# Berghojo/bmhrl

Measured on AMD Instinct MI355X. Metric: caption-train steps/sec, higher is better.
Workload: dtype bf16; 1 GPU; BMHRL warmstart step (BASELINE configs[1]): B=16/GPU Tv=256 Ta=800 L=30 V=10172 N=2 d_model=1024 H=4 dropout=0.1; global_batch=16, parallelism=dp1, launch=hip-graph

## Files before the change

bmhrl_amd/csrc/gemm.hip:

```cpp
#include <cstdlib>
#include <algorithm>
#include <type_traits>

#include "common.h"
#include "../../include/bmhrl_hip.h"

namespace {

struct GemmArgs {
  int M, N, K, batch2;
  const bf16_t* A; long lda, a_sb1, a_sb2;
  const bf16_t* B; long ldb, b_sb1, b_sb2;
  float* C; long ldc, c_sb1, c_sb2;
  bf16_t* Cb; long ldcb, cb_sb1, cb_sb2;
  int epilogue; float alpha; int relu; int accumulate;
  const float* bias;
  const float* residual; long ldr, r_sb1, r_sb2;
  const uint8_t* mask; long mask_sb1, mask_sm;
  const float* rowvec; const float* rowvec2; long rv_sb1, rv_sb2;
  const bf16_t* aux; long ldaux, aux_sb1, aux_sb2;
  float dropout_p; uint64_t seed; const uint64_t* seed_dev; long drop_sb1, drop_sb2, drop_sm;
  float* colsum; long cs_sb2, bias_sb2, cs_sb1, bias_sb1;
  int tiles_m, splits, k_per_split, vec_ok, dbg, fast_bf16, fast_pd, fast_f32, tiles_mn;
  int xcd_chunk, group_m;
// ... 586 lines not shown
}

struct GemmGroup {
  GemmArgs p0, p1, p2, p3;
  int first[5];
  int n;
};
template <int TM, int TN, bool AT, bool BT>
__global__ __launch_bounds__(256, 2) void gemm_group_kernel(const GemmGroup g) {
  const int b = (int)blockIdx.x;
  int i = 0;
  if (g.n > 1 && b >= g.first[1]) i = 1;
  if (g.n > 2 && b >= g.first[2]) i = 2;
  if (g.n > 3 && b >= g.first[3]) i = 3;
  GemmArgs p = g.p0;
  if (i == 1) p = g.p1;
  if (i == 2) p = g.p2;
  if (i == 3) p = g.p3;
  int r = b - g.first[i];
  const int bx = r % p.tiles_mn;
  r /= p.tiles_mn;
  gemm_body<TM, TN, AT, BT>(p, bx, r % p.splits, r / p.splits);
}


template <int N> struct IC { static constexpr int value = N; };
template <int I, int N, class F>
__device__ __forceinline__ void gsfor(F&& f) {
  if constexpr (I < N) {
    f(IC<I>{});
    gsfor<I + 1, N>(f);
  }
}
template <int IMM>
__device__ __forceinline__ void gemm_glds16(const char* src, char* dst) {
  __builtin_amdgcn_global_load_lds((const __attribute__((address_space(1))) void*)src,
                                   (__attribute__((address_space(3))) void*)dst, 16, IMM, 0);
}

template <int OFF>
__device__ __forceinline__ bf16x8 gemm_lds128(unsigned addr) {
  bf16x8 r;
  asm volatile("ds_read_b128 %0, %1 offset:%2" : "=v"(r) : "v"(addr), "n"(OFF));
  return r;
}
template <int OFF>
__device__ __forceinline__ bf16x4 gemm_ldstr(unsigned addr) {
  bf16x4 r;
  asm volatile("ds_read_b64_tr_b16 %0, %1 offset:%2" : "=v"(r) : "v"(addr), "n"(OFF));
  return r;
}

template <int TM, int TN, bool AT, bool BT, int NS>
__global__ __launch_bounds__(256, 2) void gemm_glds_kernel(const GemmArgs p) {
  constexpr int BM = 64 * TM, BN = 64 * TN;
  constexpr int A_BYTES = BM * BK * 2, B_BYTES = BN * BK * 2, STAGE_BYTES = A_BYTES + B_BYTES;
  constexpr int EPI_ELEMS = BM * (BN + 4) * 2;
  constexpr int SMEM_ELEMS = (NS * STAGE_BYTES / 2) > EPI_ELEMS ? (NS * STAGE_BYTES / 2) : EPI_ELEMS;

  __shared__ __attribute__((aligned(16))) bf16_t smem[SMEM_ELEMS];
  char* const sbase = reinterpret_cast<char*>(smem);
  const unsigned lds0 = (unsigned)(uintptr_t)(__attribute__((address_space(3))) char*)sbase;

  const int tid = threadIdx.x, lane = tid & 63;
  const int wave = __builtin_amdgcn_readfirstlane(tid >> 6);
  const int wm = wave >> 1, wn = wave & 1;
  const int r32 = lane & 31, h = lane >> 5;
  const int g1 = (lane >> 4) & 1, q4 = (lane & 15) >> 2, p4 = lane & 3;
  const int bz = blockIdx.z, b1 = bz / p.batch2, b2 = bz % p.batch2;
  int tile_m, tile_n;
  tile_of_block(p, (int)blockIdx.x, tile_m, tile_n);
  const int m0 = tile_m * BM, n0 = tile_n * BN;
  const char* __restrict__ Ag = reinterpret_cast<const char*>(p.A + b1 * p.a_sb1 + b2 * p.a_sb2);
  const char* __restrict__ Bg = reinterpret_cast<const char*>(p.B + b1 * p.b_sb1 + b2 * p.b_sb2);
  const int M8 = (p.M + 7) & ~7, N8 = (p.N + 7) & ~7;
  const int k_begin = blockIdx.y * p.k_per_split;
  const int k_end = min(p.K, k_begin + p.k_per_split);
  const int nk = (k_end - k_begin) / BK;
  if (nk <= 0) return;
  BMHRL_GSTAMP(0)

  constexpr int PA = A_BYTES / 1024 / 4, PB = B_BYTES / 1024 / 4;
  unsigned a_off[PA], b_off[PB];
  auto piece_off = [&](const bool trans, const int R, const int i, const int r0, const int rmax, const int rmax8, const long ld) {
    if (!trans) {
      const int row = wave * (R / 4) + 8 * i + (lane >> 3), pc = lane & 7;
      const int sc = pc ^ ((row >> 1) & 7);
      return (unsigned)((long)min(r0 + row, rmax - 1) * ld * 2 + sc * 16);
    }
    const int cpr = R / 8, rpp = 64 / cpr;
    const int krow = wave * 16 + rpp * i + lane / cpr, pc = lane % cpr;
    const int sc = pc ^ (R == 128 ? ((krow & 3) << 2) : (((krow >> 1) & 1) << 2));
    return (unsigned)((long)krow * ld * 2 + (long)min(r0 + sc * 8, rmax8 - 8) * 2);
  };
#pragma unroll
  for (int i = 0; i < PA; ++i) a_off[i] = piece_off(AT, BM, i, m0, p.M, M8, p.lda);
#pragma unroll
  for (int i = 0; i < PB; ++i) b_off[i] = piece_off(BT, BN, i, n0, p.N, N8, p.ldb);
  const long a_step = AT ? (long)BK * p.lda * 2 : (long)BK * 2, b_step = BT ? (long)BK * p.ldb * 2 : (long)BK * 2;
  const char* const a_k0 = Ag + (AT ? (long)k_begin * p.lda * 2 : (long)k_begin * 2);
  const char* const b_k0 = Bg + (BT ? (long)k_begin * p.ldb * 2 : (long)k_begin * 2);
  char* const a_dst = sbase + wave * PA * 1024;
  char* const b_dst = sbase + A_BYTES + wave * PB * 1024;
  auto stage = [&](auto st_, const int t) {
    constexpr int ST = decltype(st_)::value;
    auto sgpr_ptr = [](const char* q) {
      const uint64_t u = reinterpret_cast<uint64_t>(q);
      const uint32_t lo = __builtin_amdgcn_readfirstlane((uint32_t)u), hi = __builtin_amdgcn_readfirstlane((uint32_t)(u >> 32));
      return reinterpret_cast<const char*>(((uint64_t)hi << 32) | lo);
    };
    const char* ab = sgpr_ptr(a_k0 + (long)t * a_step);
    const char* bb = sgpr_ptr(b_k0 + (long)t * b_step);
    gsfor<0, PA>([&](auto i) {
      constexpr int I = decltype(i)::value;
      unsigned o = a_off[I];
      asm volatile("" : "+v"(o));
      gemm_glds16<0>(ab + o, a_dst + ST * STAGE_BYTES + I * 1024);
    });
    gsfor<0, PB>([&](auto i) {
      constexpr int I = decltype(i)::value;
      unsigned o = b_off[I];
      asm volatile("" : "+v"(o));
      gemm_glds16<0>(bb + o, b_dst + ST * STAGE_BYTES + I * 1024);
    });
  };

  constexpr int NA = AT ? TM : 4, NB = BT ? TN : 4;
  unsigned a_addr0[NA], b_addr0[NB];
  if constexpr (!AT) {
// ... 64 lines not shown
    read_ks(IC<1>{});
    gsfor<0, 4>([&](auto ks_) {
      constexpr int KS = decltype(ks_)::value;
      constexpr int LEFT = KS < 3 ? PER_KS : 0;
      __builtin_amdgcn_sched_barrier(0);
      bf16x8& a0 = af[KS][0];
      bf16x8& b0 = bfr[KS][0];
      bf16x8& a1 = af[KS][TM - 1];
      bf16x8& b1r = bfr[KS][TN - 1];
      if constexpr (TM == 2 && TN == 2) asm volatile("s_waitcnt lgkmcnt(%4)" : "+v"(a0), "+v"(a1), "+v"(b0), "+v"(b1r) : "n"(LEFT));
      else asm volatile("s_waitcnt lgkmcnt(%2)" : "+v"(a0), "+v"(b0) : "n"(LEFT));
      __builtin_amdgcn_sched_barrier(0);
#pragma unroll
      for (int mi = 0; mi < TM; ++mi)
#pragma unroll
        for (int ni = 0; ni < TN; ++ni)
          acc[mi][ni] = __builtin_amdgcn_mfma_f32_32x32x16_bf16(af[KS][mi], bfr[KS][ni], acc[mi][ni], 0, 0, 0);
      if constexpr (KS + 2 < 4) read_ks(IC<KS + 2>{});
    });
  };

  constexpr int PT = PA + PB;
  auto step = [&](auto st_, const int t) {
    constexpr int ST = decltype(st_)::value;
    constexpr int NXT = (ST + NS - 1) % NS;
    const bool more = t + NS - 1 < nk;
    if (more) stage(IC<NXT>{}, t + NS - 1);
    compute(st_);
    if (t + 1 < nk) {
      if (more && NS > 2) asm volatile("s_waitcnt vmcnt(%0)" ::"n"((NS - 2) * PT) : "memory");
      else asm volatile("s_waitcnt vmcnt(0)" ::: "memory");
      __builtin_amdgcn_s_barrier();
      asm volatile("" ::: "memory");
    }
  };
  gsfor<0, NS - 1>([&](auto i_) {
    if (decltype(i_)::value < nk) stage(i_, decltype(i_)::value);
  });
  BMHRL_GSTAMP(1)
  if (NS > 2 && nk > 1) asm volatile("s_waitcnt vmcnt(%0)" ::"n"((NS - 2) * PT) : "memory");
  if (NS == 2 || nk < NS - 1) asm volatile("s_waitcnt vmcnt(0)" ::: "memory");
  __builtin_amdgcn_s_barrier();
  asm volatile("" ::: "memory");
  BMHRL_GSTAMP(2)
  for (int t0 = 0; t0 < nk; t0 += NS) {
    gsfor<0, NS>([&](auto i_) {
      if (t0 + decltype(i_)::value < nk) step(i_, t0 + decltype(i_)::value);
    });
  }
  asm volatile("s_waitcnt lgkmcnt(0)" ::: "memory");
  __builtin_amdgcn_s_barrier();
  asm volatile("" ::: "memory");
  BMHRL_GSTAMP(3)
  gemm_epilogue<TM, TN, SMEM_ELEMS>(p, acc, smem, b1, b2, m0, n0, (int)blockIdx.y);
  BMHRL_GSTAMP(4)
}

template <bool AT, bool BT>
__global__ __launch_bounds__(512, 2) void gemm_glds8_kernel(const GemmArgs p) {
  constexpr int TM = 2, TN = 2, NS = 3, NW = 8;
  constexpr int BM = 128, BN = 128;
  constexpr int A_BYTES = BM * BK * 2, B_BYTES = BN * BK * 2, STAGE_BYTES = A_BYTES + B_BYTES;
  constexpr int EPI_ELEMS = BM * (BN + 4) * 2;
  constexpr int SMEM_ELEMS = (NS * STAGE_BYTES / 2) > EPI_ELEMS ? (NS * STAGE_BYTES / 2) : EPI_ELEMS;
  static_assert(4 * 64 * 256 <= SMEM_ELEMS * 2, "the partial tile of wave group 1 fits the stages");

  __shared__ __attribute__((aligned(16))) bf16_t smem[SMEM_ELEMS];
  char* const sbase = reinterpret_cast<char*>(smem);
  const unsigned lds0 = (unsigned)(uintptr_t)(__attribute__((address_space(3))) char*)sbase;

  const int tid = threadIdx.x, lane = tid & 63;
  const int wave = __builtin_amdgcn_readfirstlane(tid >> 6);
  const int grp = wave >> 2, w4 = wave & 3;
  const int wm = w4 >> 1, wn = w4 & 1;
  const int r32 = lane & 31, h = lane >> 5;
  const int g1 = (lane >> 4) & 1, q4 = (lane & 15) >> 2, p4 = lane & 3;
  const int bz = blockIdx.z, b1 = bz / p.batch2, b2 = bz % p.batch2;
  const int tile_m = blockIdx.x % p.tiles_m, tile_n = blockIdx.x / p.tiles_m;
  const int m0 = tile_m * BM, n0 = tile_n * BN;
  const char* __restrict__ Ag = reinterpret_cast<const char*>(p.A + b1 * p.a_sb1 + b2 * p.a_sb2);
  const char* __restrict__ Bg = reinterpret_cast<const char*>(p.B + b1 * p.b_sb1 + b2 * p.b_sb2);
  const int M8 = (p.M + 7) & ~7, N8 = (p.N + 7) & ~7;
  const int nk = p.K / BK;
  BMHRL_GSTAMP(0)

  constexpr int PA = A_BYTES / 1024 / NW, PB = B_BYTES / 1024 / NW;
  unsigned a_off[PA], b_off[PB];
  auto piece_off = [&](const bool trans, const int R, const int i, const int r0, const int rmax, const int rmax8, const long ld) {
    if (!trans) {
      const int row = wave * (R / NW) + 8 * i + (lane >> 3), pc = lane & 7;
      const int sc = pc ^ ((row >> 1) & 7);
      return (unsigned)((long)min(r0 + row, rmax - 1) * ld * 2 + sc * 16);
    }
    const int cpr = R / 8, rpp = 64 / cpr;
    const int krow = wave * (64 / NW) + rpp * i + lane / cpr, pc = lane % cpr;
    const int sc = pc ^ ((krow & 3) << 2);
    return (unsigned)((long)krow * ld * 2 + (long)min(r0 + sc * 8, rmax8 - 8) * 2);
  };
#pragma unroll
  for (int i = 0; i < PA; ++i) a_off[i] = piece_off(AT, BM, i, m0, p.M, M8, p.lda);
#pragma unroll
  for (int i = 0; i < PB; ++i) b_off[i] = piece_off(BT, BN, i, n0, p.N, N8, p.ldb);
  const long a_step = AT ? (long)BK * p.lda * 2 : (long)BK * 2, b_step = BT ? (long)BK * p.ldb * 2 : (long)BK * 2;
  char* const a_dst = sbase + wave * PA * 1024;
  char* const b_dst = sbase + A_BYTES + wave * PB * 1024;
  auto stage = [&](auto st_, const int t) {
    constexpr int ST = decltype(st_)::value;
    auto sgpr_ptr = [](const char* q) {
// ... 357 lines not shown
             d->r_sb2 % 4 == 0 && al(d->aux, 8) && d->ldaux % 4 == 0 && d->aux_sb1 % 4 == 0 && d->aux_sb2 % 4 == 0 &&
             al(d->bias, 16) && d->bias_sb2 % 4 == 0 && d->bias_sb1 % 4 == 0;
  a.fast_bf16 = d->Cb && !d->C && d->epilogue == BMHRL_EPI_LINEAR && !d->mask && !d->residual && !d->aux && !d->colsum &&
                !d->accumulate && al(d->Cb, 16) && d->ldcb % 8 == 0 && d->cb_sb1 % 8 == 0 && d->cb_sb2 % 8 == 0;
  static const int fast_f32_on = getenv("BMHRL_GEMM_FAST_F32") ? atoi(getenv("BMHRL_GEMM_FAST_F32")) : 1;
  const bool f32_combo = d->accumulate ? (!d->residual && d->dropout_p == 0.f && !d->Cb)
                                       : d->residual ? (d->dropout_p > 0.f || !d->Cb) : (d->dropout_p == 0.f && !d->Cb);
  a.fast_f32 = fast_f32_on && d->C && d->epilogue == BMHRL_EPI_LINEAR && !d->mask && !d->aux && !d->rowvec && !d->rowvec2 &&
               !d->relu && !d->colsum && f32_combo && a.vec_ok;
  const bool out_ok = d->Cb && !d->C && !d->residual && !d->colsum && !d->accumulate && !d->bias && al(d->Cb, 16) &&
                      d->ldcb % 8 == 0 && d->cb_sb1 % 8 == 0 && d->cb_sb2 % 8 == 0 && d->rowvec;
  a.fast_pd = (d->epilogue == BMHRL_EPI_PROB && out_ok && d->rowvec2 && (!d->mask || d->mask_sm == 0) && !d->aux) ||
              (d->epilogue == BMHRL_EPI_DSCORE && out_ok && d->aux && al(d->aux, 16) && d->ldaux % 8 == 0 &&
               d->aux_sb1 % 8 == 0 && d->aux_sb2 % 8 == 0 && (!d->mask || d->mask_sm == 0));
  const bool can_split = d->allow_split_k && d->C && !d->Cb && d->epilogue == BMHRL_EPI_LINEAR && !d->relu && !d->mask &&
                         d->dropout_p == 0.f && (!d->accumulate || d->split_ws) && !d->colsum;
  tp = tile_plan(d->M, d->N, d->K, batch, can_split);
  a.split_ws = (tp.splits > 1 && d->split_ws && d->split_ws_elems >= (int64_t)tp.splits * batch * d->M * d->N) ? d->split_ws : nullptr;
  if (tp.splits > 1 && d->accumulate && !a.split_ws) return -22;
  return 0;
}

int plan_problem(const bmhrl_gemm_desc* d, GemmArgs& a, GemmPlan& pl, int& batch) {
  TilePlan tp;
  if (const int rc = prepare(d, a, tp, batch)) return rc;
  const int TM = tp.mid || tp.big ? 2 : 1, TN = tp.big && !tp.mid ? 2 : 1;
  pl.tile = tp.mid ? TILE_128x64 : tp.big ? TILE_128 : TILE_64;
  pl.splits = tp.splits;
  pl.loop = LOOP_REG;
  pl.stages = 2;
  if (uses_glds(a, d->a_trans, d->b_trans)) {
    static const int force_ns = getenv("BMHRL_GEMM_STAGES") ? atoi(getenv("BMHRL_GEMM_STAGES")) : 0;
    const long blocks = (long)((d->M + 64 * TM - 1) / (64 * TM)) * ((d->N + 64 * TN - 1) / (64 * TN)) * batch;
    int ns = TM == 1 && tp.splits == 1 && blocks <= 448 ? 4 : 2;
    if (force_ns) ns = TM == 1 ? (force_ns >= 4 ? 4 : 2) : 2;
    pl.loop = LOOP_GLDS;
    pl.stages = ns;
    static const int w8 = getenv("BMHRL_GEMM_W8") ? atoi(getenv("BMHRL_GEMM_W8")) : 0;
    static const long w8_max = getenv("BMHRL_GEMM_W8MAX") ? atol(getenv("BMHRL_GEMM_W8MAX")) : 256;
    if (TM == 2 && TN == 2 && w8 && tp.splits == 1 && d->K >= 2 * BK && (w8 == 2 || blocks <= w8_max)) {
      pl.loop = LOOP_GLDS8;
      pl.stages = 3;
    }
  }
  pl.split_form = tp.splits == 1 ? SPLIT_NONE : a.split_ws ? SPLIT_ORDERED : SPLIT_ATOMIC;
  pl.epi_path = tp.splits == 1 && a.fast_bf16 ? EPIPATH_FAST_BF16 : tp.splits == 1 && a.fast_pd ? EPIPATH_FAST_PD : EPIPATH_GENERIC;
  if (tp.splits != 1 || pl.loop == LOOP_GLDS8) a.fast_f32 = 0;
  pl.fast_f32 = a.fast_f32;
  pl.vec_ok = a.vec_ok;
  pl.ordered_colsum = bmhrl_deterministic() && a.colsum != nullptr;
  return 0;
}

int group_prepare(const bmhrl_gemm_desc* d, int n, GemmGroup& g, int& total) {
  GemmArgs* ps[4] = {&g.p0, &g.p1, &g.p2, &g.p3};
  bool same = n > 1;
  total = 0;
  for (int i = 0; i < n; ++i) {
    GemmPlan pl;
    int batch;
    if (const int rc = plan_problem(d + i, *ps[i], pl, batch)) return rc;
    GemmArgs& p = *ps[i];
    same = same && pl.tile == TILE_64 && pl.loop == LOOP_REG && d[i].a_trans == d[0].a_trans && d[i].b_trans == d[0].b_trans &&
           pl.split_form != SPLIT_ORDERED && !pl.ordered_colsum;
    p.tiles_m = (p.M + 63) / 64;
    p.tiles_mn = p.tiles_m * ((p.N + 63) / 64);
    p.splits = pl.splits;
    p.dbg = 0;
    const int ktiles = (p.K + BK - 1) / BK;
    p.k_per_split = ((ktiles + pl.splits - 1) / pl.splits) * BK;
    g.first[i] = total;
    total += p.tiles_mn * pl.splits * batch;
  }
  return same ? 1 : 0;
}
}

extern "C" int bmhrl_gemm_plan(const bmhrl_gemm_desc* d, int32_t plan[8]) {
  GemmArgs a;
  GemmPlan pl;
  int batch;
  if (const int rc = plan_problem(d, a, pl, batch)) return rc;
  if (plan) {
    plan[0] = pl.loop; plan[1] = pl.tile; plan[2] = pl.stages; plan[3] = pl.splits;
    plan[4] = pl.split_form; plan[5] = pl.epi_path; plan[6] = pl.vec_ok; plan[7] = pl.ordered_colsum;
  }
  return 0;
}

extern "C" int bmhrl_gemm_f32_fast_path(const bmhrl_gemm_desc* d) {
  GemmArgs a;
  GemmPlan pl;
  int batch;
  if (const int rc = plan_problem(d, a, pl, batch)) return rc;
  return pl.fast_f32;
}

extern "C" int bmhrl_gemm_group_plan(const bmhrl_gemm_desc* d, int32_t n) {
  BMHRL_CHECK_ARG(d && n >= 1);
  int launches = 0;
  for (int i = 0; i < n; i += 4) {
    GemmGroup g;
    int total;
    const int rc = group_prepare(d + i, n - i < 4 ? n - i : 4, g, total);
    if (rc < 0) return rc;
    launches += rc;
  }
  return launches;
}

void gemm_trace_dump(const GemmArgs& a, hipStream_t stream) {
#ifdef BMHRL_GEMM_TRACE
  if (getenv("BMHRL_GEMM_TRACE")) {
    long long hh[2][8];
    (void)hipStreamSynchronize(stream);
    (void)hipMemcpyFromSymbol(hh, HIP_SYMBOL(g_gemm_trace), sizeof(hh));
    for (int w = 0; w < 2; ++w)
      fprintf(stderr, "gemm trace (%s block, M %d N %d K %d): setup %lld  first tile %lld  loop %lld  epilogue %lld  total %lld\n",
              w ? "last" : "first", a.M, a.N, a.K, hh[w][1] - hh[w][0], hh[w][2] - hh[w][1], hh[w][3] - hh[w][2], hh[w][4] - hh[w][3],
              hh[w][4] - hh[w][0]);
  }
#else
  (void)a; (void)stream;
#endif
}

extern "C" int bmhrl_gemm(const bmhrl_gemm_desc* d, bmhrl_stream_t stream) {
  GemmArgs a;
  GemmPlan pl;
  int batch;
  if (const int rc = plan_problem(d, a, pl, batch)) return rc;
  GemmArgs full = a;
  if (pl.ordered_colsum) a.colsum = nullptr;
  hipError_t e;
  if (pl.tile == TILE_128x64) e = launch<2, 1>(a, pl, d->a_trans, d->b_trans, batch, (hipStream_t)stream);
  else if (pl.tile == TILE_128) e = launch<2, 2>(a, pl, d->a_trans, d->b_trans, batch, (hipStream_t)stream);
  else e = launch<1, 1>(a, pl, d->a_trans, d->b_trans, batch, (hipStream_t)stream);
  if (e == hipSuccess && pl.ordered_colsum) {
    hipLaunchKernelGGL(colsum_ordered_kernel, dim3((unsigned)((full.N + 63) / 64)), dim3(1024), 0, (hipStream_t)stream, full, d->batch1);
    e = hipGetLastError();
  }
  if (e == hipSuccess && pl.split_form == SPLIT_ORDERED) {
    GemmArgs r = a;
    r.splits = pl.splits;
    const int ktiles = (a.K + BK - 1) / BK, tiles_per_split = (ktiles + pl.splits - 1) / pl.splits;
    const int n_live = (ktiles + tiles_per_split - 1) / tiles_per_split;
    const long total = (long)batch * a.M * a.N;
    hipLaunchKernelGGL(splitk_reduce_kernel, dim3((unsigned)std::min<long>((total + 255) / 256, 2048)), dim3(256), 0, (hipStream_t)stream, r, batch,
                       n_live);
    e = hipGetLastError();
  }
  gemm_trace_dump(a, (hipStream_t)stream);
  return hip_status(e);
}

extern "C" int bmhrl_gemm_group(const bmhrl_gemm_desc* d, int32_t n, bmhrl_stream_t stream) {
  BMHRL_CHECK_ARG(d && n >= 1);
  if (n > 4) {
    for (int i = 0; i < n; i += 4)
      if (const int rc = bmhrl_gemm_group(d + i, n - i < 4 ? n - i : 4, stream)) return rc;
    return 0;
  }
  GemmGroup g;
  int total;
  const int same = group_prepare(d, n, g, total);
  if (same < 0) return same;
  if (!same) {
    for (int i = 0; i < n; ++i)
      if (const int rc = bmhrl_gemm(d + i, stream)) return rc;
    return 0;
  }
  GemmArgs* ps[4] = {&g.p0, &g.p1, &g.p2, &g.p3};
  for (int i = n; i < 5; ++i) g.first[i] = total;
  for (int i = n; i < 4; ++i) *ps[i] = g.p0;
  g.n = n;
  dim3 grid((unsigned)total), block(256);
  const hipStream_t s = (hipStream_t)stream;
  if (!d[0].a_trans && !d[0].b_trans) hipLaunchKernelGGL((gemm_group_kernel<1, 1, false, false>), grid, block, 0, s, g);
  else if (!d[0].a_trans && d[0].b_trans) hipLaunchKernelGGL((gemm_group_kernel<1, 1, false, true>), grid, block, 0, s, g);
  else if (d[0].a_trans && !d[0].b_trans) hipLaunchKernelGGL((gemm_group_kernel<1, 1, true, false>), grid, block, 0, s, g);
  else hipLaunchKernelGGL((gemm_group_kernel<1, 1, true, true>), grid, block, 0, s, g);
  return hip_status(hipGetLastError());
}
```

bmhrl_amd/functional.py:

```python
from __future__ import annotations

import math
import itertools
import os
import weakref
from typing import Optional

import torch

from . import ops
from .ops import pad8

_BF16 = torch.bfloat16


class ShadowCache:

    def __init__(self):
        self.w = {}
        self.b = {}
        self.split = {}
        self.epoch = 0

    def invalidate(self):
# ... 426 lines not shown
    scale = 1.0 / math.sqrt(dk)
    Skp = pad8(Sk)
    pstr = (H * Sq * Skp, Sq * Skp)
    fused = (FUSED_SCORES_BWD and stats[0] == "flash" and ops.attention_bwd_scores256_ok(Sq, Sk, dk, msq)
             and all(v % 8 == 0 for v in (ldq, ldk, ldv, q_off, k_off, v_off)))
    if fused:
        P = torch.empty(B, H, Sq, Skp, dtype=_BF16, device=dev)
        dS = torch.empty(B, H, Sq, Skp, dtype=_BF16, device=dev)
        ops.attention_bwd_scores256(Qb, ldq, Kb, ldk, Vb, ldv, dOb, D, stats[1], stats[2], mask, msb, P, dS, Skp, B, H, Sq, Sk,
                                    scale, q_off=q_off, k_off=k_off, v_off=v_off)
        _attn_grad_products(P, dS, pstr, dOb, Qb, q_off, ldq, Kb, k_off, ldk, dQb, dq_off, lddq, dKb, dk_off, lddk, dVb, dv_off,
                            lddv, B, H, Sq, Sk, dk, Skp, csq, csk, csv)
        return
    delta = torch.empty(B, H, Sq, device=dev)
    ops.attn_delta(dOb, D, Ob, D, delta, B, H, Sq, dk, scale=1.0 - p_drop)
    if stats[0] == "flash":
        P = _padded_bf16(B * H * Sq, Sk, dev).view(B, H, Sq, Skp)
        ops.gemm(Qb, Kb, Sq, Sk, dk, lda=ldq, ldb=ldk, a_off=q_off, b_off=k_off, batch=(B, H), a_strides=(Sq * ldq, dk),
                 b_strides=(Sk * ldk, dk), C_bf16=P, ldcb=Skp, cb_strides=pstr, epilogue=ops.EPI_PROB, alpha=scale,
                 mask=mask, mask_sb1=msb, mask_sm=msq, rowvec=stats[1], rowvec2=stats[2], rv_strides=(H * Sq, Sq))
    else:
        P = stats[1]
    dS = _padded_bf16(B * H * Sq, Sk, dev).view(B, H, Sq, Skp)
    ops.gemm(dOb, Vb, Sq, Sk, dk, lda=D, ldb=ldv, b_off=v_off, batch=(B, H), a_strides=(Sq * D, dk),
             b_strides=(Sk * ldv, dk), C_bf16=dS, ldcb=Skp, cb_strides=pstr, epilogue=ops.EPI_DSCORE, alpha=scale,
             rowvec=delta, rv_strides=(H * Sq, Sq), aux=P, ldaux=Skp, aux_strides=pstr, mask=mask, mask_sb1=msb, mask_sm=msq)
    _attn_grad_products(P, dS, pstr, dOb, Qb, q_off, ldq, Kb, k_off, ldk, dQb, dq_off, lddq, dKb, dk_off, lddk, dVb, dv_off, lddv,
                        B, H, Sq, Sk, dk, Skp, csq, csk, csv)


def _attn_grad_products(P, dS, pstr, dOb, Qb, q_off, ldq, Kb, k_off, ldk, dQb, dq_off, lddq, dKb, dk_off, lddk, dVb, dv_off, lddv,
                        B, H, Sq, Sk, dk, Skp, csq, csk, csv):
    D = H * dk
    ops.gemm(P, dOb, Sk, dk, Sq, lda=Skp, ldb=D, a_trans=True, b_trans=True, batch=(B, H), a_strides=pstr,
             b_strides=(Sq * D, dk), C_bf16=dVb, ldcb=lddv, cb_off=dv_off, cb_strides=(Sk * lddv, dk), **csv)
    ops.gemm(dS, Qb, Sk, dk, Sq, lda=Skp, ldb=ldq, b_off=q_off, a_trans=True, b_trans=True, batch=(B, H), a_strides=pstr,
             b_strides=(Sq * ldq, dk), C_bf16=dKb, ldcb=lddk, cb_off=dk_off, cb_strides=(Sk * lddk, dk), **csk)
    ops.gemm(dS, Kb, Sq, dk, Sk, lda=Skp, ldb=ldk, b_off=k_off, b_trans=True, batch=(B, H), a_strides=pstr,
             b_strides=(Sk * ldk, dk), C_bf16=dQb, ldcb=lddq, cb_off=dq_off, cb_strides=(Sq * lddq, dk), **csq)


ORDERED_DX = os.environ.get("BMHRL_ORDERED_DX", "1") == "1"


def _split_ws(M, N, K, batch, device):
    if not ORDERED_DX:
        return None
    n = ops.gemm_splits(M, N, K, batch)
    return SCRATCH.f32(n * batch * M * N, device=device, zero=False) if n > 1 else None


def _linear_bwd(dyb, ldy, rows, N, xb, ldx, K, wb, *, need_dw, need_db, need_dx, dx_f32=None, dx_bf16=None, lddxb=0,
                dx_epilogue=ops.EPI_LINEAR, dx_alpha=1.0, dx_aux=None, ldaux=0, dx_drop=0.0, dx_seed=0,
                dy_off=0, x_off=0, w_off=0, dx_accumulate=False, dx_colsum=None, dx_split_k=False, leaf=None):
    dev = dyb.device
    dw = db = None
    if need_dw:
        dw = SCRATCH.f32(N, K, device=dev, zero=not ops.gemm_overwrites(N, K, rows))
        ops.gemm(dyb, xb, N, K, rows, lda=ldy, ldb=ldx, a_off=dy_off, b_off=x_off, a_trans=True, b_trans=True, C_f32=dw, ldc=K,
                 allow_split_k=True, defer=leaf)
    if need_db:
        db = SCRATCH.f32(N, device=dev)
        ops.colsum_bf16(dyb, ldy, db, True, rows, N, dy_off=dy_off)
    if need_dx:
        ws = _split_ws(rows, K, N, 1, dev) if dx_split_k else None
        ops.gemm(dyb, wb, rows, K, N, lda=ldy, ldb=wb.shape[1], a_off=dy_off, b_off=w_off, b_trans=True, C_f32=dx_f32,
                 ldc=K, C_bf16=dx_bf16, ldcb=lddxb, epilogue=dx_epilogue, alpha=dx_alpha, aux=dx_aux, ldaux=ldaux,
                 dropout_p=dx_drop, seed=dx_seed, seed_dev=SEEDS.dev, accumulate=dx_accumulate, colsum=dx_colsum,
                 allow_split_k=dx_split_k, split_ws=ws)
    return dw, db


def _row_stride(t, cols):
    if t.dim() < 2 or t.shape[-1] != cols or t.stride(-1) != 1:
        return None
    for i in range(t.dim() - 2):
        if t.shape[i] != 1 and t.stride(i) != t.stride(i + 1) * t.shape[i + 1]:
            return None
    return t.stride(-2) if t.stride(-2) >= cols else None


def _cast_dy(dy, rows, N, p_drop, seed, want_db, ld=None):
    dev = dy.device
    ld = N if ld is None else ld
    dyb = SCRATCH.bf16(rows, N, dev)
    if want_db:
        db = SCRATCH.f32(N, device=dev)
        ops.cast_colsum_bf16(dy, ld, dyb, dyb.shape[1], rows, N, db, dropout_p=p_drop, seed=seed, seed_dev=SEEDS.dev)
        return dyb, db
    ops.cast_bf16(dy, ld, dyb, dyb.shape[1], rows, N, dropout_p=p_drop, seed=seed, seed_dev=SEEDS.dev)
    return dyb, None


class MHAFn(torch.autograd.Function):

    @staticmethod
    def forward(ctx, x, kv_in, ln_w, ln_b, wq, bq, wk, bk, wv, bv, wo, bo, mask, H, p_drop, residual, kv_cache=None,
                emit_bf16=False):
        dev = x.device
        B, Sq, dq = x.shape
        D = wq.shape[0]
        dk = D // H
        rows_q = B * Sq
        x = x.contiguous()
        self_att = kv_in is None
        has_ln = ln_w is not None
        ldx = pad8(dq)
        mean = rstd = None
        if has_ln:
            xb = SCRATCH.bf16(rows_q, dq, dev)
            mean = torch.empty(rows_q, device=dev)
            rstd = torch.empty(rows_q, device=dev)
            ops.layernorm_fwd(x, ln_w.detach(), ln_b.detach(), xb, ldx, None, mean, rstd, rows_q, dq)
# ... 14 lines not shown
            _, Sk, dkv = kv_in.shape
            rows_k = B * Sk
            w_q = SHADOWS.weight(wq)
            Qb = torch.empty(rows_q, D, dtype=_BF16, device=dev)
            ops.gemm(xb, w_q, rows_q, D, dq, lda=ldx, ldb=w_q.shape[1], C_bf16=Qb, ldcb=D, bias=bq.detach())
            KV = kv_cache.get((id(wk), id(wv))) if kv_cache is not None else None
            kvb = None
            if KV is None:
                kv_in = kv_in.contiguous()
                kvb = SCRATCH.memo_bf16(kv_in, rows_k, dkv)
                w_kv = SHADOWS.weight(wk, wv)
                KV = torch.empty(rows_k, 2 * D, dtype=_BF16, device=dev)
                ops.gemm(kvb, w_kv, rows_k, 2 * D, dkv, lda=kvb.shape[1], ldb=w_kv.shape[1], C_bf16=KV, ldcb=2 * D,
                         bias=SHADOWS.bias(bk, bv))
                if kv_cache is not None:
                    kv_cache[(id(wk), id(wv))] = KV
            Kb = Vb = KV
            q_off, k_off, v_off, ldq, ldk = 0, 0, D, D, 2 * D
        Ob, stats = _attn_core_fwd(Qb, q_off, ldq, Kb, k_off, ldk, Vb, v_off, ldk, m8, msb, msq, B, H, Sq, Sk, dk, p_drop, s_attn)
        w_o = SHADOWS.weight(wo)
        y = torch.empty(B, Sq, dq, device=dev)
        yb = SCRATCH.bf16(rows_q, dq, dev) if (emit_bf16 and SCRATCH.armed) else None
        ops.gemm(Ob, w_o, rows_q, dq, D, lda=D, ldb=w_o.shape[1], C_f32=y, ldc=dq, bias=bo.detach(),
                 residual=x if residual else None, ldr=dq, dropout_p=p_drop, seed=s_res, seed_dev=SEEDS.dev,
                 C_bf16=yb, ldcb=yb.shape[1] if yb is not None else 0)
        if yb is not None:
            SCRATCH.offer_bf16(y, rows_q, dq, yb)
        ctx.save_for_backward(x, ln_w, mean, rstd, xb, kvb, Qb, Kb, Ob, m8, *stats[1:], wq, wk, wv, wo)
        ctx.cfg = (B, H, Sq, Sk, dq, dkv, D, dk, p_drop, residual, self_att, has_ln, stats[0], msb, msq, s_attn, s_res,
                   q_off, k_off, v_off, ldq, ldk)
        return y

    @staticmethod
    def backward(ctx, dy):
        (B, H, Sq, Sk, dq, dkv, D, dk, p_drop, residual, self_att, has_ln, kind, msb, msq, s_attn, s_res, q_off, k_off, v_off,
         ldq, ldk) = ctx.cfg
        saved = ctx.saved_tensors
        x, ln_w, mean, rstd, xb, kvb, Qb, Kb, Ob, m8 = saved[:10]
        n_stats = 2 if kind == "flash" else 1
        stats = (kind,) + tuple(saved[10:10 + n_stats])
        wq, wk, wv, wo = saved[10 + n_stats:]
        Vb = Kb
        dev = dy.device
        rows_q, rows_k = B * Sq, B * Sk
        ldx = pad8(dq)
        need = ctx.needs_input_grad
        ld_dy = None if dy.is_contiguous() or (residual and has_ln) else _row_stride(dy, dq)
        if ld_dy is None:
            dy = dy.contiguous()
        keep = 1.0 / (1.0 - p_drop) if p_drop > 0 else 1.0
        dyb, dbo = _cast_dy(dy, rows_q, dq, p_drop, s_res, need[11], ld=ld_dy)
        dOb = torch.empty(rows_q, D, dtype=_BF16, device=dev)
        w_o = SHADOWS.weight(wo)
        leaf = [] if max(rows_q, rows_k) < 2048 else None
        dwo, _ = _linear_bwd(dyb, ldx, rows_q, dq, Ob, D, D, w_o, need_dw=need[10], need_db=False, need_dx=True,
                             dx_bf16=dOb, lddxb=D, dx_drop=p_drop, dx_seed=s_attn, leaf=leaf)
        del keep
        if self_att:
            dQKV = torch.empty(rows_q, 3 * D, dtype=_BF16, device=dev)
            dQb = dKb = dVb = dQKV
            lddq = lddk = 3 * D
        else:
            dQb = torch.empty(rows_q, D, dtype=_BF16, device=dev)
            dKV = torch.empty(rows_k, 2 * D, dtype=_BF16, device=dev)
            dKb = dVb = dKV
            lddq, lddk = D, 2 * D
        need_bq, need_bkv = need[5], need[7] or need[9]
        if self_att:
            db_all = SCRATCH.f32(3 * D, device=dev) if (need_bq or need_bkv) else None
            tq = tk = tv = None
            if db_all is not None:
                tq, tk, tv = (db_all, 0), (db_all, D), (db_all, 2 * D)
        else:
            db_qq = SCRATCH.f32(D, device=dev) if need_bq else None
            db_kv = SCRATCH.f32(2 * D, device=dev) if need_bkv else None
            tq = (db_qq, 0) if need_bq else None
            tk = (db_kv, 0) if need_bkv else None
            tv = (db_kv, D) if need_bkv else None
        _attn_core_bwd(dOb, Ob, stats, Qb, q_off, ldq, Kb, k_off, ldk, Vb, v_off, ldk, dQb, q_off, lddq, dKb, k_off, lddk,
                       dVb, v_off, lddk, m8, msb, msq, B, H, Sq, Sk, dk, p_drop, db_q=tq, db_k=tk, db_v=tv)
        dxn = torch.empty(rows_q, dq, device=dev) if (need[0] or (has_ln and (need[2] or need[3]))) else None
        dwq = dbq = dwk = dbk = dwv = dbv = dkv_in = None
        if self_att:
            w_qkv = SHADOWS.weight(wq, wk, wv)
            need_w = need[4] or need[6] or need[8]
            dw, _ = _linear_bwd(dQKV, 3 * D, rows_q, 3 * D, xb, ldx, dq, w_qkv, need_dw=need_w, need_db=False,
                                need_dx=dxn is not None, dx_f32=dxn, leaf=leaf)
            db = db_all
            if dw is not None:
                dwq, dwk, dwv = dw[:D], dw[D:2 * D], dw[2 * D:]
            if db is not None:
                dbq, dbk, dbv = db[:D], db[D:2 * D], db[2 * D:]
        else:
            w_q = SHADOWS.weight(wq)
            w_kv = SHADOWS.weight(wk, wv)
            dwq, _ = _linear_bwd(dQb, D, rows_q, D, xb, ldx, dq, w_q, need_dw=need[4], need_db=False,
                                 need_dx=dxn is not None, dx_f32=dxn, leaf=leaf)
            dbq = db_qq
            if need[1]:
                dkv_in = torch.empty(B, Sk, dkv, device=dev)
            dw, _ = _linear_bwd(dKV, 2 * D, rows_k, 2 * D, kvb, kvb.shape[1], dkv, w_kv, need_dw=need[6] or need[8],
                                need_db=False, need_dx=need[1], dx_f32=dkv_in, leaf=leaf)
            db = db_kv
            if dw is not None:
                dwk, dwv = dw[:D], dw[D:]
            if db is not None:
                dbk, dbv = db[:D], db[D:]
        if leaf:
            ops.gemm_flush(leaf)
        dx = dlnw = dlnb = None
        if has_ln:
            if dxn is not None:
                dx = torch.empty(B, Sq, dq, device=dev)
                dlnw = SCRATCH.f32(dq, device=dev) if need[2] else None
                dlnb = SCRATCH.f32(dq, device=dev) if need[3] else None
                ops.layernorm_bwd(dxn, x, ln_w, mean, rstd, dx, dy if residual else None, dlnw, dlnb, rows_q, dq)
        elif need[0]:
            dx = dxn.view(B, Sq, dq)
            if residual:
                dx = dx + dy
        return (dx, dkv_in, dlnw, dlnb, dwq, dbq, dwk, dbk, dwv, dbv, dwo, dbo, None, None, None, None, None, None)


FUSED_ATTN_BWD = os.environ.get("BMHRL_FUSED_ATTN_BWD", "1") != "0"


class MemAttnFn(torch.autograd.Function):

    @staticmethod
    def forward(ctx, x, mem, ln_w, ln_b, wq, bq, wk, bk, wv, bv, wo, bo, mask, H, p_drop, emit_bf16=False):
        dev = x.device
        B, L, dq = x.shape
        self_att = mem is None
        Sk, dm = (L, dq) if self_att else mem.shape[1:]
        D = wq.shape[0]
        dk = D // H
        rows = B * L
        x = x.contiguous()
        ldx, dmp, Skp = pad8(dq), pad8(dm), pad8(Sk)
        scale = 1.0 / math.sqrt(dk)
        xb = SCRATCH.bf16(rows, dq, dev)
        mean = torch.empty(rows, device=dev)
        rstd = torch.empty(rows, device=dev)
        ops.layernorm_fwd(x, ln_w.detach(), ln_b.detach(), xb, ldx, None, mean, rstd, rows, dq)
        s_attn, s_res = SEEDS.next(), SEEDS.next()
        w_q, w_k, w_v, w_o = SHADOWS.weight(wq), SHADOWS.weight(wk), SHADOWS.weight(wv), SHADOWS.weight(wo)
        Qb = torch.empty(rows, D, dtype=_BF16, device=dev)
        ops.gemm(xb, w_q, rows, D, dq, lda=ldx, ldb=w_q.shape[1], C_bf16=Qb, ldcb=D, bias=bq.detach())
        memb = xb if self_att else SCRATCH.memo_bf16(mem, B * Sk, dm)
        zeros = torch.zeros if dmp != dm else torch.empty
        Qp = zeros(rows, H * dmp, dtype=_BF16, device=dev)
        ops.gemm(Qb, w_k, rows, dm, dk, lda=D, ldb=w_k.shape[1], b_trans=True, batch=(1, H), a_strides=(0, dk),
                 b_strides=(0, dk * w_k.shape[1]), C_bf16=Qp, ldcb=H * dmp, cb_strides=(0, dmp))
        m8, msb, msq = _mask_u8(mask)
        Cx = zeros(rows, H * dmp, dtype=_BF16, device=dev)
# ... 511 lines not shown
        dOb = torch.empty(rows_q, D, dtype=_BF16, device=dev)
        ops.cast_bf16(dO.contiguous(), D, dOb, D, rows_q, D, dropout_p=p_drop, seed=seed, seed_dev=SEEDS.dev)
        dQb = torch.empty(rows_q, D, dtype=_BF16, device=dev)
        dKV = torch.empty(rows_k, 2 * D, dtype=_BF16, device=dev)
        _attn_core_bwd(dOb, Ob, stats, Qb, 0, D, KV, 0, 2 * D, KV, D, 2 * D, dQb, 0, D, dKV, 0, 2 * D, dKV, D, 2 * D,
                       m8, msb, msq, B, H, Sq, Sk, dk, p_drop)
        need = ctx.needs_input_grad
        dq = dQb.float().view(B, Sq, D) if need[0] else None
        dk_ = dKV[:, :D].float().view(B, Sk, D) if need[1] else None
        dv = dKV[:, D:].float().view(B, Sk, D) if need[2] else None
        return dq, dk_, dv, None, None, None


class FFNFn(torch.autograd.Function):

    @staticmethod
    def forward(ctx, x, ln_w, ln_b, w1, b1, w2, b2, p_drop):
        dev = x.device
        B, S, d = x.shape
        rows = B * S
        dff = w1.shape[0]
        x = x.contiguous()
        ldx = pad8(d)
        xb = SCRATCH.bf16(rows, d, dev)
        mean = torch.empty(rows, device=dev)
        rstd = torch.empty(rows, device=dev)
        ops.layernorm_fwd(x, ln_w.detach(), ln_b.detach(), xb, ldx, None, mean, rstd, rows, d)
        s_in, s_res = SEEDS.next(), SEEDS.next()
        wb1, wb2 = SHADOWS.weight(w1), SHADOWS.weight(w2)
        hb = SCRATCH.bf16(rows, dff, dev)
        ops.gemm(xb, wb1, rows, dff, d, lda=ldx, ldb=wb1.shape[1], C_bf16=hb, ldcb=hb.shape[1], bias=b1.detach(), relu=True,
                 dropout_p=p_drop, seed=s_in, seed_dev=SEEDS.dev)
        y = torch.empty(B, S, d, device=dev)
        ops.gemm(hb, wb2, rows, d, dff, lda=hb.shape[1], ldb=wb2.shape[1], C_f32=y, ldc=d, bias=b2.detach(), residual=x, ldr=d,
                 dropout_p=p_drop, seed=s_res, seed_dev=SEEDS.dev)
        ctx.save_for_backward(x, ln_w, mean, rstd, xb, hb, w1, w2)
        ctx.cfg = (B, S, d, dff, p_drop, s_in, s_res)
        return y

    @staticmethod
    def backward(ctx, dy):
        B, S, d, dff, p_drop, s_in, s_res = ctx.cfg
        x, ln_w, mean, rstd, xb, hb, w1, w2 = ctx.saved_tensors
        dev = dy.device
        rows = B * S
        ldx = pad8(d)
        need = ctx.needs_input_grad
        dy = dy.contiguous()
        dyb, db2 = _cast_dy(dy, rows, d, p_drop, s_res, need[6])
        wb1, wb2 = SHADOWS.weight(w1), SHADOWS.weight(w2)
        dzb = SCRATCH.bf16(rows, dff, dev)
        keep = 1.0 / (1.0 - p_drop) if p_drop > 0 else 1.0
        db1 = SCRATCH.f32(dff, device=dev) if need[4] else None
        dw2, _ = _linear_bwd(dyb, ldx, rows, d, hb, hb.shape[1], dff, wb2, need_dw=need[5], need_db=False, need_dx=True,
                             dx_bf16=dzb, lddxb=dzb.shape[1], dx_epilogue=ops.EPI_RELU_BWD, dx_alpha=keep, dx_aux=hb,
                             ldaux=hb.shape[1], dx_colsum=db1)
        dxn = torch.empty(rows, d, device=dev)
        dw1, _ = _linear_bwd(dzb, dzb.shape[1], rows, dff, xb, ldx, d, wb1, need_dw=need[3], need_db=False, need_dx=True,
                             dx_f32=dxn)
        dx = torch.empty(B, S, d, device=dev)
        dlnw = SCRATCH.f32(d, device=dev) if need[1] else None
        dlnb = SCRATCH.f32(d, device=dev) if need[2] else None
        ops.layernorm_bwd(dxn, x, ln_w, mean, rstd, dx, dy, dlnw, dlnb, rows, d)
        return dx, dlnw, dlnb, dw1, db1, dw2, db2, None


class LinearFn(torch.autograd.Function):

    @staticmethod
    def forward(ctx, x, w, b, relu, p_drop):
        dev = x.device
        shp = x.shape
        K = shp[-1]
        rows = x.numel() // K
        N = w.shape[0]
        x2 = x.contiguous().view(rows, K)
        xb = SCRATCH.memo_bf16(x2, rows, K)
        wb = SHADOWS.weight(w)
        y = torch.empty(rows, N, device=dev)
        seed = SEEDS.next()
        ops.gemm(xb, wb, rows, N, K, lda=xb.shape[1], ldb=wb.shape[1], C_f32=y, ldc=N, bias=None if b is None else b.detach(),
                 relu=relu, dropout_p=p_drop, seed=seed, seed_dev=SEEDS.dev)
        ctx.save_for_backward(xb, w, y if (relu or p_drop > 0) else None)
        ctx.cfg = (shp, rows, N, K, relu, p_drop, seed, b is not None)
        return y.view(*shp[:-1], N)

    @staticmethod
    def backward(ctx, dy):
        shp, rows, N, K, relu, p_drop, seed, has_b = ctx.cfg
        xb, w, y = ctx.saved_tensors
        dev = dy.device
        need = ctx.needs_input_grad
        dy2 = dy.contiguous().view(rows, N)
        if y is not None:
            keep = 1.0 / (1.0 - p_drop) if p_drop > 0 else 1.0
            dy2 = torch.where(y != 0, dy2 * keep, torch.zeros_like(dy2)) if relu else None
            if dy2 is None:
                dy2 = dy.contiguous().view(rows, N)
        drop = p_drop if not relu else 0.0
        dyb, db = _cast_dy(dy2, rows, N, drop, seed, has_b and need[2])
        wb = SHADOWS.weight(w)
        dx = torch.empty(rows, K, device=dev) if need[0] else None
        dw, _ = _linear_bwd(dyb, dyb.shape[1], rows, N, xb, xb.shape[1], K, wb, need_dw=need[1], need_db=False,
                            need_dx=need[0], dx_f32=dx)
        return (dx.view(shp) if dx is not None else None), dw, db, None, None


class Conv1dSameFn(torch.autograd.Function):

    @staticmethod
    def _operand(w):
        co, ci, k = w.shape
# ... 673 lines not shown
```

profiles/summarize.py:

```python
#!/usr/bin/env python3
import collections
import csv
import glob
import sys

d, steps = sys.argv[1], float(sys.argv[2])
stats = list(csv.DictReader(open(glob.glob(d + "/**/*_kernel_stats.csv", recursive=True)[0])))
tot = sum(float(r["TotalDurationNs"]) for r in stats)
print(f"total kernel time {tot / 1e6:.2f} ms over {steps:g} steps = {tot / 1e6 / steps:.3f} ms/step\n")
print("| kernel | calls/step | avg us | ms/step | % |\n|---|---|---|---|---|")
for r in stats[:40]:
    print(f"| {r['Name'][:100]} | {float(r['Calls']) / steps:.1f} | {float(r['AverageNs']) / 1e3:.1f} | "
          f"{float(r['TotalDurationNs']) / 1e6 / steps:.3f} | {float(r['Percentage']):.1f} |")
tr = glob.glob(d + "/**/*_kernel_trace.csv", recursive=True)
if tr:
    agg = collections.defaultdict(list)
    for r in csv.DictReader(open(tr[0])):
        n = r["Kernel_Name"]
        if "gemm_kernel" in n or "gemm_glds_kernel" in n or "attn_" in n:
            if "gemm_glds_kernel" in n:
                short = "gemm_glds" + n.split("gemm_glds_kernel")[1].split("(")[0]
            elif "gemm_kernel" in n:
                short = "gemm" + n.split("gemm_kernel")[1].split("(")[0]
            else:
                short = "attn_" + n.split("attn_")[1].split("(")[0][:40]
            agg[(short, int(r["Grid_Size_X"]) // int(r["Workgroup_Size_X"]), r["Grid_Size_Y"], r["Grid_Size_Z"])].append(
                (int(r["End_Timestamp"]) - int(r["Start_Timestamp"])) / 1e3)
    print("\n| kernel | blocks x | y | z | calls/step | avg us | ms/step |\n|---|---|---|---|---|---|---|")
    for k, v in sorted(agg.items(), key=lambda kv: -sum(kv[1]))[:50]:
        print(f"| {k[0]} | {k[1]} | {k[2]} | {k[3]} | {len(v) / steps:.1f} | {sum(v) / len(v):.1f} | {sum(v) / steps / 1e3:.3f} |")
```

Measured before the change: 206.7 steps/s (one step = one B=16 batch on one GPU; whole-job aggregate over all GPUs).

## Batch deferred weight-gradient GEMMs into grouped glds kernel launches

```diff
diff --git a/bmhrl_amd/csrc/gemm.hip b/bmhrl_amd/csrc/gemm.hip
--- a/bmhrl_amd/csrc/gemm.hip
+++ b/bmhrl_amd/csrc/gemm.hip
@@ -662,7 +662,7 @@
 }
 
 template <int TM, int TN, bool AT, bool BT, int NS>
-__global__ __launch_bounds__(256, 2) void gemm_glds_kernel(const GemmArgs p) {
+__device__ __forceinline__ void gemm_glds_body(const GemmArgs& p, const int bx, const int by, const int bz) {
   constexpr int BM = 64 * TM, BN = 64 * TN;
   constexpr int A_BYTES = BM * BK * 2, B_BYTES = BN * BK * 2, STAGE_BYTES = A_BYTES + B_BYTES;
   constexpr int EPI_ELEMS = BM * (BN + 4) * 2;
@@ -677,14 +677,14 @@
   const int wm = wave >> 1, wn = wave & 1;
   const int r32 = lane & 31, h = lane >> 5;
   const int g1 = (lane >> 4) & 1, q4 = (lane & 15) >> 2, p4 = lane & 3;
-  const int bz = blockIdx.z, b1 = bz / p.batch2, b2 = bz % p.batch2;
+  const int b1 = bz / p.batch2, b2 = bz % p.batch2;
   int tile_m, tile_n;
-  tile_of_block(p, (int)blockIdx.x, tile_m, tile_n);
+  tile_of_block(p, bx, tile_m, tile_n);
   const int m0 = tile_m * BM, n0 = tile_n * BN;
   const char* __restrict__ Ag = reinterpret_cast<const char*>(p.A + b1 * p.a_sb1 + b2 * p.a_sb2);
   const char* __restrict__ Bg = reinterpret_cast<const char*>(p.B + b1 * p.b_sb1 + b2 * p.b_sb2);
   const int M8 = (p.M + 7) & ~7, N8 = (p.N + 7) & ~7;
-  const int k_begin = blockIdx.y * p.k_per_split;
+  const int k_begin = by * p.k_per_split;
   const int k_end = min(p.K, k_begin + p.k_per_split);
   const int nk = (k_end - k_begin) / BK;
   if (nk <= 0) return;
@@ -855,8 +855,29 @@
   __builtin_amdgcn_s_barrier();
   asm volatile("" ::: "memory");
   BMHRL_GSTAMP(3)
-  gemm_epilogue<TM, TN, SMEM_ELEMS>(p, acc, smem, b1, b2, m0, n0, (int)blockIdx.y);
+  gemm_epilogue<TM, TN, SMEM_ELEMS>(p, acc, smem, b1, b2, m0, n0, by);
   BMHRL_GSTAMP(4)
+}
+
+template <int TM, int TN, bool AT, bool BT, int NS>
+__global__ __launch_bounds__(256, 2) void gemm_glds_kernel(const GemmArgs p) {
+  gemm_glds_body<TM, TN, AT, BT, NS>(p, (int)blockIdx.x, (int)blockIdx.y, (int)blockIdx.z);
+}
+
+template <int TM, int TN, bool AT, bool BT, int NS>
+__global__ __launch_bounds__(256, 2) void gemm_glds_group_kernel(const GemmGroup g) {
+  const int b = (int)blockIdx.x;
+  int i = 0;
+  if (g.n > 1 && b >= g.first[1]) i = 1;
+  if (g.n > 2 && b >= g.first[2]) i = 2;
+  if (g.n > 3 && b >= g.first[3]) i = 3;
+  GemmArgs p = g.p0;
+  if (i == 1) p = g.p1;
+  if (i == 2) p = g.p2;
+  if (i == 3) p = g.p3;
+  int r = b - g.first[i];
+  const int bx = r % p.tiles_mn;
+  gemm_glds_body<TM, TN, AT, BT, NS>(p, bx, 0, r / p.tiles_mn);
 }
 
 template <bool AT, bool BT>
@@ -1320,9 +1341,15 @@
   return 0;
 }
 
+constexpr int GLDS_GROUP_MIN_TILES = 192;
+enum { GROUP_NONE = 0, GROUP_REG = 1, GROUP_GLDS = 2 };
+
 int group_prepare(const bmhrl_gemm_desc* d, int n, GemmGroup& g, int& total) {
   GemmArgs* ps[4] = {&g.p0, &g.p1, &g.p2, &g.p3};
-  bool same = n > 1;
+  static const bool tile_forced = getenv("BMHRL_GEMM_TILE") && atoi(getenv("BMHRL_GEMM_TILE")) != 0;
+  bool same = n > 1, glds = n > 1 && !tile_forced;
+  int batches[4];
+  long big_tiles = 0;
   total = 0;
   for (int i = 0; i < n; ++i) {
     GemmPlan pl;
@@ -1331,6 +1358,10 @@
     GemmArgs& p = *ps[i];
     same = same && pl.tile == TILE_64 && pl.loop == LOOP_REG && d[i].a_trans == d[0].a_trans && d[i].b_trans == d[0].b_trans &&
            pl.split_form != SPLIT_ORDERED && !pl.ordered_colsum;
+    glds = glds && pl.loop == LOOP_GLDS && pl.tile != TILE_128x64 && pl.splits == 1 && d[i].a_trans && d[i].b_trans && p.C && !p.Cb &&
+           p.epilogue == BMHRL_EPI_LINEAR && !pl.ordered_colsum && p.M >= 128 && p.N >= 128 && p.K % BK == 0;
+    batches[i] = batch;
+    big_tiles += (long)((p.M + 127) / 128) * ((p.N + 127) / 128) * batch;
     p.tiles_m = (p.M + 63) / 64;
     p.tiles_mn = p.tiles_m * ((p.N + 63) / 64);
     p.splits = pl.splits;
@@ -1340,7 +1371,19 @@
     g.first[i] = total;
     total += p.tiles_mn * pl.splits * batch;
   }
-  return same ? 1 : 0;
+  if (same) return GROUP_REG;
+  if (!glds || big_tiles < GLDS_GROUP_MIN_TILES || big_tiles > (1l << 30)) return GROUP_NONE;
+  total = 0;
+  for (int i = 0; i < n; ++i) {
+    GemmArgs& p = *ps[i];
+    p.tiles_m = (p.M + 127) / 128;
+    p.tiles_mn = p.tiles_m * ((p.N + 127) / 128);
+    p.xcd_chunk = p.group_m = 0;
+    p.k_per_split = p.K;
+    g.first[i] = total;
+    total += p.tiles_mn * batches[i];
+  }
+  return GROUP_GLDS;
 }
 }
 
@@ -1372,7 +1415,7 @@
     int total;
     const int rc = group_prepare(d + i, n - i < 4 ? n - i : 4, g, total);
     if (rc < 0) return rc;
-    launches += rc;
+    launches += rc != GROUP_NONE;
   }
   return launches;
 }
@@ -1444,7 +1487,8 @@
   g.n = n;
   dim3 grid((unsigned)total), block(256);
   const hipStream_t s = (hipStream_t)stream;
-  if (!d[0].a_trans && !d[0].b_trans) hipLaunchKernelGGL((gemm_group_kernel<1, 1, false, false>), grid, block, 0, s, g);
+  if (same == GROUP_GLDS) hipLaunchKernelGGL((gemm_glds_group_kernel<2, 2, true, true, 2>), grid, block, 0, s, g);
+  else if (!d[0].a_trans && !d[0].b_trans) hipLaunchKernelGGL((gemm_group_kernel<1, 1, false, false>), grid, block, 0, s, g);
   else if (!d[0].a_trans && d[0].b_trans) hipLaunchKernelGGL((gemm_group_kernel<1, 1, false, true>), grid, block, 0, s, g);
   else if (d[0].a_trans && !d[0].b_trans) hipLaunchKernelGGL((gemm_group_kernel<1, 1, true, false>), grid, block, 0, s, g);
   else hipLaunchKernelGGL((gemm_group_kernel<1, 1, true, true>), grid, block, 0, s, g);
diff --git a/bmhrl_amd/functional.py b/bmhrl_amd/functional.py
--- a/bmhrl_amd/functional.py
+++ b/bmhrl_amd/functional.py
@@ -502,13 +502,15 @@
 
 def _linear_bwd(dyb, ldy, rows, N, xb, ldx, K, wb, *, need_dw, need_db, need_dx, dx_f32=None, dx_bf16=None, lddxb=0,
                 dx_epilogue=ops.EPI_LINEAR, dx_alpha=1.0, dx_aux=None, ldaux=0, dx_drop=0.0, dx_seed=0,
-                dy_off=0, x_off=0, w_off=0, dx_accumulate=False, dx_colsum=None, dx_split_k=False, leaf=None):
+                dy_off=0, x_off=0, w_off=0, dx_accumulate=False, dx_colsum=None, dx_split_k=False, leaf=None,
+                leaf_unsplit_only=False):
     dev = dyb.device
     dw = db = None
     if need_dw:
-        dw = SCRATCH.f32(N, K, device=dev, zero=not ops.gemm_overwrites(N, K, rows))
+        once = ops.gemm_overwrites(N, K, rows)
+        dw = SCRATCH.f32(N, K, device=dev, zero=not once)
         ops.gemm(dyb, xb, N, K, rows, lda=ldy, ldb=ldx, a_off=dy_off, b_off=x_off, a_trans=True, b_trans=True, C_f32=dw, ldc=K,
-                 allow_split_k=True, defer=leaf)
+                 allow_split_k=True, defer=leaf if (once or not leaf_unsplit_only) else None)
     if need_db:
         db = SCRATCH.f32(N, device=dev)
         ops.colsum_bf16(dyb, ldy, db, True, rows, N, dy_off=dy_off)
@@ -629,9 +631,10 @@
         dyb, dbo = _cast_dy(dy, rows_q, dq, p_drop, s_res, need[11], ld=ld_dy)
         dOb = torch.empty(rows_q, D, dtype=_BF16, device=dev)
         w_o = SHADOWS.weight(wo)
-        leaf = [] if max(rows_q, rows_k) < 2048 else None
+        leaf = []
+        long_block = max(rows_q, rows_k) >= 2048
         dwo, _ = _linear_bwd(dyb, ldx, rows_q, dq, Ob, D, D, w_o, need_dw=need[10], need_db=False, need_dx=True,
-                             dx_bf16=dOb, lddxb=D, dx_drop=p_drop, dx_seed=s_attn, leaf=leaf)
+                             dx_bf16=dOb, lddxb=D, dx_drop=p_drop, dx_seed=s_attn, leaf=leaf, leaf_unsplit_only=long_block)
         del keep
         if self_att:
             dQKV = torch.empty(rows_q, 3 * D, dtype=_BF16, device=dev)
@@ -662,7 +665,7 @@
             w_qkv = SHADOWS.weight(wq, wk, wv)
             need_w = need[4] or need[6] or need[8]
             dw, _ = _linear_bwd(dQKV, 3 * D, rows_q, 3 * D, xb, ldx, dq, w_qkv, need_dw=need_w, need_db=False,
-                                need_dx=dxn is not None, dx_f32=dxn, leaf=leaf)
+                                need_dx=dxn is not None, dx_f32=dxn, leaf=leaf, leaf_unsplit_only=long_block)
             db = db_all
             if dw is not None:
                 dwq, dwk, dwv = dw[:D], dw[D:2 * D], dw[2 * D:]
@@ -672,12 +675,12 @@
             w_q = SHADOWS.weight(wq)
             w_kv = SHADOWS.weight(wk, wv)
             dwq, _ = _linear_bwd(dQb, D, rows_q, D, xb, ldx, dq, w_q, need_dw=need[4], need_db=False,
-                                 need_dx=dxn is not None, dx_f32=dxn, leaf=leaf)
+                                 need_dx=dxn is not None, dx_f32=dxn, leaf=leaf, leaf_unsplit_only=long_block)
             dbq = db_qq
             if need[1]:
                 dkv_in = torch.empty(B, Sk, dkv, device=dev)
             dw, _ = _linear_bwd(dKV, 2 * D, rows_k, 2 * D, kvb, kvb.shape[1], dkv, w_kv, need_dw=need[6] or need[8],
-                                need_db=False, need_dx=need[1], dx_f32=dkv_in, leaf=leaf)
+                                need_db=False, need_dx=need[1], dx_f32=dkv_in, leaf=leaf, leaf_unsplit_only=long_block)
             db = db_kv
             if dw is not None:
                 dwk, dwv = dw[:D], dw[D:]
@@ -1295,12 +1298,14 @@
         dzb = SCRATCH.bf16(rows, dff, dev)
         keep = 1.0 / (1.0 - p_drop) if p_drop > 0 else 1.0
         db1 = SCRATCH.f32(dff, device=dev) if need[4] else None
+        leaf = []
         dw2, _ = _linear_bwd(dyb, ldx, rows, d, hb, hb.shape[1], dff, wb2, need_dw=need[5], need_db=False, need_dx=True,
                              dx_bf16=dzb, lddxb=dzb.shape[1], dx_epilogue=ops.EPI_RELU_BWD, dx_alpha=keep, dx_aux=hb,
-                             ldaux=hb.shape[1], dx_colsum=db1)
+                             ldaux=hb.shape[1], dx_colsum=db1, leaf=leaf, leaf_unsplit_only=True)
         dxn = torch.empty(rows, d, device=dev)
         dw1, _ = _linear_bwd(dzb, dzb.shape[1], rows, dff, xb, ldx, d, wb1, need_dw=need[3], need_db=False, need_dx=True,
-                             dx_f32=dxn)
+                             dx_f32=dxn, leaf=leaf, leaf_unsplit_only=True)
+        ops.gemm_flush(leaf)
         dx = torch.empty(B, S, d, device=dev)
         dlnw = SCRATCH.f32(d, device=dev) if need[1] else None
         dlnb = SCRATCH.f32(d, device=dev) if need[2] else None
diff --git a/profiles/summarize.py b/profiles/summarize.py
--- a/profiles/summarize.py
+++ b/profiles/summarize.py
@@ -17,8 +17,10 @@
     agg = collections.defaultdict(list)
     for r in csv.DictReader(open(tr[0])):
         n = r["Kernel_Name"]
-        if "gemm_kernel" in n or "gemm_glds_kernel" in n or "attn_" in n:
-            if "gemm_glds_kernel" in n:
+        if "gemm_kernel" in n or "gemm_glds_kernel" in n or "gemm_glds_group_kernel" in n or "attn_" in n:
+            if "gemm_glds_group_kernel" in n:
+                short = "gemm_glds_group" + n.split("gemm_glds_group_kernel")[1].split("(")[0]
+            elif "gemm_glds_kernel" in n:
                 short = "gemm_glds" + n.split("gemm_glds_kernel")[1].split("(")[0]
             elif "gemm_kernel" in n:
                 short = "gemm" + n.split("gemm_kernel")[1].split("(")[0]
```

Measured after the change: 208.4 steps/s (one step = one B=16 batch on one GPU; whole-job aggregate over all GPUs) (median of 6 runs). No clear change (+0.8%).
